# nayuki/DEFLATE-library-Java

Measured on AMD Instinct MI355X. Metric: input MiB/s (compress+decompress), higher is better.
Workload: dtype u8

## Files before the change

deflate-library-java_amd/csrc/capi/ndfl_capi.cpp:

```cpp
#include "../../../include/ndfl.h"
#include "../hip/deflate_kernels.hip"
#include "../hip/deflate_split.hip"
#include "../hip/lz77_kernels.hip"
#include "../hip/strategy_kernels.hip"
#include "../hip/inflate_kernels.hip"

#include <hip/hip_runtime.h>
#include <string.h>
#include <stdio.h>
#include <algorithm>
#include <stdlib.h>
#include <vector>
#include <functional>
#include <map>

namespace {

struct DevBuf {
    void* p = nullptr;
    size_t cap = 0;
    hipError_t ensure(size_t n) {
        if (n <= cap) return hipSuccess;
        if (p) { hipFree(p); p = nullptr; cap = 0; }
        size_t want = n < 4096 ? 4096 : n;
// ... 229 lines not shown
    HIPCHK(c->d_status.ensure(nch * sizeof(uint64_t)));
    HIPCHK(c->d_ticket.ensure(64));
    HIPCHK(c->d_edge_w.ensure(2ull * nch * sizeof(uint64_t)));
    HIPCHK(c->d_edge_v.ensure(2ull * nch * sizeof(uint32_t)));
    if (crc_inout) { HIPCHK(c->d_crc.ensure(nch * sizeof(uint32_t))); HIPCHK(c->d_crc1.ensure(64)); }
    HIPCHK(hipMemsetAsync(c->d_status.p, 0, nch * sizeof(uint64_t), s));
    HIPCHK(hipMemsetAsync(c->d_ticket.p, 0, 64, s));

    Args a;
    a.in = d_data; a.n = len; a.chunk_len = chunk_len; a.nchunks = nch;
    a.prev_byte = prev_byte; a.hist_enabled = hist_limit > 0; a.final_last = final_flag ? 1 : 0;
    a.rle = rle; a.dynamic = dyn; a.base_bit = start_bitpos;
    a.parent_len = c->parent_len ? c->parent_len : chunk_len;
    a.out = d_out; a.status = c->d_status.as<uint64_t>(); a.ticket = c->d_ticket.as<uint32_t>();
    a.edge_w = c->d_edge_w.as<uint64_t>(); a.edge_v = c->d_edge_v.as<uint32_t>();
    a.chunk_bits = c->cb_out;
    a.crc_raw = crc_inout ? c->d_crc.as<uint32_t>() : nullptr;
    a.crc_tab = c->d_tabs.as<uint32_t>();
    a.crc_x = c->d_tabs.as<uint32_t>() + 1024;
    a.prof = nullptr;
    const bool prof = c->knobs.deflate_profile;
    if (prof) { HIPCHK(hipMalloc(&a.prof, (size_t)nch * 128)); HIPCHK(hipMemsetAsync(a.prof, 0, (size_t)nch * 128, s)); }
    a.hist_out = nullptr; a.codes = nullptr; a.chunk_off = nullptr;
    {
        static int ncu = 0;
        if (!ncu && hipDeviceGetAttribute(&ncu, hipDeviceAttributeMultiprocessorCount, c->device) != hipSuccess) ncu = 0;
        a.pf_dist = c->knobs.deflate_pf ? 2u * (uint32_t)ncu : 0u;
    }
    const bool split = !c->knobs.deflate_fused && !prof;
    uint64_t* d_total = nullptr;
    if (split) {
        HIPCHK(c->d_hist.ensure((size_t)nch * HREC * 4));
        HIPCHK(c->d_codes.ensure((size_t)nch * CREC * 4));
        HIPCHK(c->d_off.ensure((size_t)nch * 8 + 64 + (size_t)((nch + SCAN_TILE - 1) / SCAN_TILE) * 8));
        a.hist_out = c->d_hist.as<uint32_t>();
        a.codes = c->d_codes.as<uint32_t>();
        a.chunk_off = c->d_off.as<uint64_t>();
        d_total = c->d_off.as<uint64_t>() + nch;
    }
    a.c0 = 0;
    HIPCHK(hipEventRecord(c->ev0, s));
    if (split) {
        hipLaunchKernelGGL(ndfl_deflate_hist_kernel, dim3(nch), dim3(1024), 0, s, a);
        HIPCHK(hipGetLastError());
        hipLaunchKernelGGL(ndfl_deflate_codes_kernel, dim3(nch), dim3(64), 0, s, a);
        HIPCHK(hipGetLastError());
        const uint32_t ntile = (nch + SCAN_TILE - 1) / SCAN_TILE;
        uint64_t* d_part = c->d_off.as<uint64_t>() + nch + 8;
        hipLaunchKernelGGL(ndfl_deflate_offsets_sum_kernel, dim3(ntile), dim3(SCAN_T), 0, s, (const uint64_t*)a.status,
                           nch, d_part);
        HIPCHK(hipGetLastError());
        hipLaunchKernelGGL(ndfl_deflate_offsets_kernel, dim3(ntile), dim3(SCAN_T), 0, s, (const uint64_t*)a.status, nch,
                           (uint64_t)start_bitpos, c->d_off.as<uint64_t>(), d_total, (const uint64_t*)d_part);
        HIPCHK(hipGetLastError());
        hipLaunchKernelGGL(ndfl_deflate_emit_kernel, dim3(nch), dim3(1024), 0, s, a);
    } else {
        hipLaunchKernelGGL(ndfl_deflate_chunks_kernel, dim3(nch), dim3(1024), 0, s, a);
    }
    HIPCHK(hipGetLastError());
    HIPCHK(hipEventRecord(c->ev1, s));
    const uint32_t ne = 2 * nch;
    hipLaunchKernelGGL(ndfl_edge_fixup_kernel, dim3((ne + 255) / 256), dim3(256), 0, s,
                       (const uint64_t*)a.edge_w, (const uint32_t*)a.edge_v, ne, d_out);
    HIPCHK(hipGetLastError());
    if (crc_inout) {
        HIPCHK(launch_crc_combine(c, s, (const uint32_t*)a.crc_raw, nch, chunk_len, len, c->d_crc1.as<uint32_t>()));
        HIPCHK(hipMemcpyAsync(c->h_pinned + 4, c->d_crc1.p, 4, hipMemcpyDeviceToHost, s));
    }
    if (split) HIPCHK(hipMemcpyAsync(c->h_pinned, d_total, 8, hipMemcpyDeviceToHost, s));
    else HIPCHK(hipMemcpyAsync(c->h_pinned, a.status + (nch - 1), 8, hipMemcpyDeviceToHost, s));
    HIPCHK(hipStreamSynchronize(s));
    float ms = 0;
    hipEventElapsedTime(&ms, c->ev0, c->ev1);
    c->last_ms = ms;
    c->deflate_ms = ms;
    if (prof) {
        std::vector<uint64_t> h((size_t)nch * 16);
        HIPCHK(hipMemcpy(h.data(), a.prof, (size_t)nch * 128, hipMemcpyDeviceToHost));
        hipFree(a.prof);
        double sum[7] = {0}, tmin = 1e300, tmax = 0, sub[6] = {0};
        uint64_t nsub = 0;
        for (uint32_t k = 0; k < nch; k++) {
            const uint64_t* q = &h[k * 16];
            for (int p = 0; p < 7; p++) sum[p] += (double)(q[p + 1] - q[p]);
            tmin = std::min(tmin, (double)q[0]); tmax = std::max(tmax, (double)q[7]);
            if (q[8]) {
                const uint64_t t[7] = {q[2], q[8], q[9], q[10], q[11], q[12], q[13]};
                for (int p = 0; p < 6; p++) sub[p] += (double)(t[p + 1] - t[p]);
                nsub++;
            }
        }
        if (nsub)
            fprintf(stderr, "[ndfl] deflate codes sub-phases (us/chunk): trim %.2f pm(lit,dist) %.2f canon %.2f cl-rle %.2f "
                    "pm(cl) %.2f canon(cl) %.2f\n", sub[0] / nsub / 100, sub[1] / nsub / 100, sub[2] / nsub / 100,
                    sub[3] / nsub / 100, sub[4] / nsub / 100, sub[5] / nsub / 100);
        fprintf(stderr, "[ndfl] deflate phases (us/chunk): load+crc %.2f hist %.2f codes %.2f bits+scan %.2f emit %.2f "
                "lookback %.2f store %.2f; span %.2f ms\n", sum[0] / nch / 100, sum[1] / nch / 100, sum[2] / nch / 100,
                sum[3] / nch / 100, sum[4] / nch / 100, sum[5] / nch / 100, sum[6] / nch / 100, (tmax - tmin) / 1e5);
    }
    uint64_t st;
    memcpy(&st, c->h_pinned, 8);
    const uint64_t end_bits = st & ST_VAL;
    *out_end_bits = end_bits;
    const uint64_t nbytes = (end_bits + 7) / 8;
    if (crc_inout) {
        uint32_t raw = c->h_pinned[4];
        uint32_t dc = ~(crc_multmodp(crc_x8n(len), 0xFFFFFFFFu) ^ raw);
        *crc_inout = ndfl_crc32_combine(*crc_inout, dc, len);
    }
// ... 673 lines not shown
```

deflate-library-java_amd/csrc/hip/deflate_kernels.hip:

```cpp
#include "ndfl_common.hpp"

namespace {

constexpr int DT = 1024;
constexpr int NW = DT / 64;
constexpr int MAX_CHUNK = 65536;
constexpr int OUTW = 18600;

constexpr uint64_t ST_AGG = 1ull << 62;
constexpr uint64_t ST_PRE = 2ull << 62;
constexpr uint64_t ST_VAL = (1ull << 62) - 1;

constexpr int SCR_HLIT = 0;
constexpr int SCR_HDIST = SCR_HLIT + 288 * 4;
constexpr int SCR_LAST = SCR_HDIST + 32 * 4;
constexpr int SCR_KEY = SCR_LAST + 1024;
constexpr int SCR_LF = SCR_KEY + 288 * 4;
constexpr int SCR_LS = SCR_LF + 288 * 4;
constexpr int SCR_PFA = SCR_LS + 288 * 4;
constexpr int SCR_PFB = SCR_PFA + 304 * 4;
constexpr int SCR_MF = SCR_PFB + 304 * 4;
constexpr int SCR_MPK = SCR_MF + 608 * 4;
constexpr int SCR_LVL = SCR_MPK + 15 * 20 * 4;
constexpr int SCR_LEN = SCR_LVL + 16 * 4;
// ... 415 lines not shown

__device__ __forceinline__ void block_store(const uint32_t* obuf, uint64_t P, uint64_t S, uint32_t c, uint32_t* out,
                                            uint64_t* edge_w, uint32_t* edge_v) {
    const int tid = threadIdx.x;
    const uint32_t sh = (uint32_t)(P & 31);
    const uint32_t nw = (uint32_t)((sh + S + 31) >> 5);
    const uint64_t W0 = P >> 5;
    auto outw = [&](uint32_t k) -> uint32_t {
        const uint32_t cur = obuf[k];
        const uint32_t prv = k ? obuf[k - 1] : 0u;
        return sh ? (cur << sh) | (prv >> (32 - sh)) : cur;
    };
    for (uint32_t k = (uint32_t)tid + 1; k + 1 < nw; k += DT) out[W0 + k] = outw(k);
    if (tid == 0) {
        edge_w[2 * c] = W0;
        edge_v[2 * c] = outw(0);
        edge_w[2 * c + 1] = W0 + nw - 1;
        edge_v[2 * c + 1] = nw > 1 ? outw(nw - 1) : 0u;
    }
}

}

template <int MODE, class PS>
__device__ __forceinline__ void deflate_chunk(const Args& a, uint32_t* obuf, PS& ps, uint32_t* hl4 = nullptr,
                                              uint32_t* ctab = nullptr) {
    char* scr = (char*)obuf;
    uint32_t* hlit = (uint32_t*)(scr + SCR_HLIT);
    uint32_t* hdist = (uint32_t*)(scr + SCR_HDIST);
    uint8_t* lastb = (uint8_t*)(scr + SCR_LAST);
    uint32_t* misc = (uint32_t*)(scr + SCR_MISC);

    const int tid = threadIdx.x;
    const int lane = tid & 63, wid = tid >> 6;

    const uint64_t tp0 = wall_clock64();
    if (MODE == MODE_FUSED) {
        if (tid == 0) ps.chunk = atomicAdd(a.ticket, 1u);
    } else {
        if (tid == 0) ps.chunk = a.c0 + blockIdx.x;
    }
    if (MODE == MODE_FUSED) {
        if (tid < 288) hlit[tid] = 0;
        if (tid < 32) hdist[tid] = 0;
    } else if (MODE == MODE_HIST) {
        for (int k = tid; k < HCOPY * HSTR; k += DT) hl4[k] = 0;
        if (a.crc_raw) ctab[tid] = a.crc_tab[tid];
    }
    __syncthreads();
    const uint32_t c = ps.chunk;
    const uint64_t cs = (uint64_t)c * a.chunk_len;
    const uint32_t len_c = (uint32_t)min((uint64_t)a.chunk_len, a.n - cs);
    const bool is_final = a.final_last && (c + 1 == a.nchunks);
    const uint8_t* src = a.in + cs;

    uint32_t w[16];
    const uint32_t t0 = (uint32_t)tid * 64;
    const int vcnt = (int)min(64u, len_c > t0 ? len_c - t0 : 0u);
    if (vcnt == 64 && (((uintptr_t)(src + t0)) & 15) == 0) {
        const u32x4* p = (const u32x4*)(src + t0);
#pragma unroll
        for (int k = 0; k < 4; k++) {
            u32x4 v = __builtin_nontemporal_load(p + k);
            w[4 * k] = v.x; w[4 * k + 1] = v.y; w[4 * k + 2] = v.z; w[4 * k + 3] = v.w;
        }
    } else {
#pragma unroll
        for (int k = 0; k < 16; k++) {
            uint32_t x = 0;
#pragma unroll
            for (int b = 0; b < 4; b++) {
                int i = 4 * k + b;
                if (i < vcnt) x |= (uint32_t)src[t0 + i] << (8 * b);
            }
            w[k] = x;
        }
    }
    if (vcnt > 0) {
        uint32_t lv = w[15] >> 24;
        if (vcnt < 64) {
#pragma unroll
            for (int i = 0; i < 64; i++) if (i == vcnt - 1) lv = (w[i >> 2] >> (8 * (i & 3))) & 0xFFu;
// ... 20 lines not shown
#pragma unroll
            for (int i = 0; i < 64; i++)
                if (i >= nfull * 4 && i < vcnt) cr = T0[(cr ^ (w[i >> 2] >> (8 * (i & 3)))) & 0xFF] ^ (cr >> 8);
        }
        uint32_t contrib = 0;
        if (vcnt > 0) {
            const uint32_t after = len_c - (t0 + (uint32_t)vcnt);
            const uint32_t q = after & 63, k64 = after >> 6;
            uint32_t sh = a.crc_x[64 + k64];
            if (q) sh = crc_multmodp(a.crc_x[q], sh);
            contrib = crc_multmodp(sh, cr);
        }
        contrib = wave_xor(contrib);
        if (lane == 0) ps.crcAcc[wid] = contrib;
    }
    __syncthreads();
    if (MODE != MODE_EMIT && a.crc_raw && tid == 0) {
        uint32_t x = 0;
        for (int k = 0; k < NW; k++) x ^= ps.crcAcc[k];
        a.crc_raw[c] = x;
    }

    const uint64_t tp1 = wall_clock64();
    uint32_t pfv = 0;
    auto prefetch_next = [&]() {
        const uint64_t cn = (uint64_t)c + a.pf_dist;
        if (a.pf_dist && cn < a.nchunks && tid < 512) {
            const uint64_t off = cn * a.chunk_len + (uint64_t)tid * 128;
            if (off < a.n) pfv = a.in[off];
        }
    };
    const bool has_prev0 = (cs % a.parent_len != 0) ? true : (c > 0) ? (a.hist_enabled != 0) : (a.prev_byte >= 0);
    const uint32_t prev0 = (c > 0) ? (uint32_t)src[-1] : (uint32_t)(a.prev_byte & 0xFF);
    uint64_t F = 0;
    if (vcnt > 0) {
        uint32_t prev = tid > 0 ? (uint32_t)lastb[tid - 1] : 0u;
        if (!a.rle) {
            F = vcnt == 64 ? ~0ull : ((1ull << vcnt) - 1);
        } else {
#pragma unroll
            for (int k = 0; k < 16; k++) {
                const uint32_t x = w[k] ^ ((w[k] << 8) | (k ? (w[k - 1] >> 24) : prev));
                const uint32_t hb = ((((x & 0x7F7F7F7Fu) + 0x7F7F7F7Fu) | x) & 0x80808080u) >> 7;
                F |= (uint64_t)(((hb * 0x00204081u) >> 21) & 0xFu) << (4 * k);
            }
            if (tid == 0) F |= 1ull;
            if (vcnt < 64) F &= (1ull << vcnt) - 1;
        }
    }
    const uint32_t firstStart = F ? t0 + (uint32_t)__builtin_ctzll(F) : 0xFFFFFFFFu;
    const uint32_t nextStart = min(block_excl_suffix_min<NW>(firstStart, 0xFFFFFFFFu, ps.scan32), len_c);

    auto lead_of = [&](uint32_t gpos, uint32_t v) -> uint32_t {
        if (!a.rle) return 1u;
        if (gpos == 0) return (has_prev0 && prev0 == v) ? 0u : 1u;
        return 1u;
    };
    uint32_t mpx = 0xFFFFu;
    if (vcnt > 0) {
        mpx = nextStart - t0;
        if (a.rle && tid == 0 && (F & 1) && lead_of(0, w[0] & 0xFFu) == 0) mpx |= 1u << 31;
    }
    uint64_t LM = 0, LG = 0;
    uint32_t ce = 0;
    if (vcnt > 0) {
        const uint32_t mq = mpx & 0xFFFFu;
        const uint64_t wl = F | (mq < 64 ? 1ull << mq : 0ull);
        const uint64_t wh = (mq >= 64 && mq < 67) ? 1ull << (mq - 64) : 0ull;
        const uint64_t e1 = (wl >> 1) | (wh << 63), e2 = (wl >> 2) | (wh << 62), e3 = (wl >> 3) | (wh << 61);
        uint64_t r3 = F & ~e1 & ~e2 & e3;
        LG = F & ~(e1 | e2 | e3);
        if ((mpx >> 31) && (r3 & 1ull)) { r3 &= ~1ull; LG |= 1ull; }
        const uint64_t r2 = (F & ~e1 & e2) | r3;
        const uint64_t r1 = (F & e1) | r2;
        LM = r1 | (r2 << 1) | (r3 << 2);
        ce = (uint32_t)(r2 >> 63) + (uint32_t)((r3 >> 62) & 1ull) + (uint32_t)(r3 >> 63);
    }
#define NDFL_FOR_GROUPS_L(...)                                                                         \
    _Pragma("unroll 1") for (int o_ = 0; o_ < 8; o_++) {                                               \
        const uint32_t lm_ = (uint32_t)(LM >> (8 * o_)) & 0xFFu;                                      \
        const uint32_t lg_ = (uint32_t)(LG >> (8 * o_)) & 0xFFu;                                      \
        if (!__any((lm_ | lg_) != 0)) continue;                                                        \
        const bool o1_ = o_ & 1, o2_ = o_ & 2, o4_ = o_ & 4;                                           \
        const uint32_t a0_ = o1_ ? w[2] : w[0], a1_ = o1_ ? w[6] : w[4];                               \
        const uint32_t a2_ = o1_ ? w[10] : w[8], a3_ = o1_ ? w[14] : w[12];                            \
        const uint32_t b0_ = o1_ ? w[3] : w[1], b1_ = o1_ ? w[7] : w[5];                               \
        const uint32_t b2_ = o1_ ? w[11] : w[9], b3_ = o1_ ? w[15] : w[13];                            \
        const uint32_t gw0_ = o4_ ? (o2_ ? a3_ : a2_) : (o2_ ? a1_ : a0_);                             \
        const uint32_t gw1_ = o4_ ? (o2_ ? b3_ : b2_) : (o2_ ? b1_ : b0_);                             \
        const bool anyL_ = __any(lg_ != 0);                                                            \
        __VA_ARGS__                                                                                    \
    }
#define NDFL_BYTE(j) ((((j) < 4 ? gw0_ : gw1_) >> (8 * ((j) & 3))) & 0xFFu)
#define NDFL_LMASK(j) ((uint32_t)((int32_t)(lm_ << (31 - (j))) >> 31))
#define NDFL_RUN_L(j, ...)                                                                             \
    if ((lg_ >> (j)) & 1) {                                                                            \
        const int i_ = 8 * o_ + (j);                                                                   \
        const uint32_t v = NDFL_BYTE(j);                                                               \
        const uint32_t gpos = t0 + (uint32_t)i_;                                                       \
        const uint64_t rest_ = i_ < 63 ? (F >> (i_ + 1)) : 0ull;                                       \
        const uint32_t pend = rest_ ? gpos + 1 + (uint32_t)__builtin_ctzll(rest_) : nextStart;         \
        __VA_ARGS__                                                                                    \
    }

    uint32_t* hl = hlit;
    uint32_t* hd = hdist;
    if (MODE == MODE_HIST) { hl = hl4 + (tid & (HCOPY - 1)) * HSTR; hd = hl + 288; }
    if (MODE == MODE_HIST) {
        asm volatile("" :: "v"(prev0));
        prefetch_next();
    }
    if (MODE != MODE_EMIT) {
    NDFL_FOR_GROUPS_L({
_Pragma("unroll")
        for (int j = 0; j < 8; j++)
            if ((lm_ >> j) & 1) atomicAdd(&hl[NDFL_BYTE(j)], 1u);
        if (!anyL_) continue;
_Pragma("unroll")
        for (int j = 0; j < 8; j++) {
            NDFL_RUN_L(j, {
                const uint32_t lead = lead_of(gpos, v);
                const uint32_t R = pend - gpos - lead;
                const uint32_t n258 = R / 258, m = R % 258;
                const uint32_t nlit = lead + (m < 3 ? m : 0);
                if (nlit) atomicAdd(&hl[v], nlit);
                if (n258) atomicAdd(&hl[285], n258);
                uint32_t nd = n258;
                if (m >= 3) {
                    uint32_t sym, ne, ex; run_sym(m, sym, ne, ex);
                    atomicAdd(&hl[sym], 1u);
                    nd++;
                }
                if (nd) atomicAdd(&hd[0], nd);
            })
        }
    })
    if (ce) atomicAdd(&hl[w[15] >> 24], ce);
    if (tid == 0) {
        atomicAdd(&hl[256], 1u);
        if (a.dynamic && len_c == 0) atomicAdd(&hl[0], 1u);
    }
    __syncthreads();
    }
    if (MODE == MODE_HIST) {
        uint32_t* h = a.hist_out + (uint64_t)c * HREC;
        if (tid < HREC) {
            uint32_t v = 0;
_Pragma("unroll")
            for (int k = 0; k < HCOPY; k++) v += hl4[k * HSTR + tid];
            h[tid] = v;
        }
        asm volatile("" :: "v"(pfv));
        return;
    }

    const uint64_t tp2 = wall_clock64();
    uint32_t packedLo = 0, packedHi = 0;
    if constexpr (MODE == MODE_FUSED) {
        build_block_codes(a.dynamic != 0, scr, ps, a.prof ? a.prof + (uint64_t)c * 16 + 8 : nullptr);
        packedLo = misc[4]; packedHi = misc[5];
    } else {
        const uint32_t* rec = a.codes + (uint64_t)c * CREC;
        if (tid < 288) ps.litCode[tid] = rec[CREC_LIT + tid];
        else if (tid < 320) ps.distCode[tid - 288] = rec[CREC_DIST + tid - 288];
        if (tid == 0) ps.hdrBits = rec[CREC_META];
    }
    __syncthreads();

    const uint64_t tp3 = wall_clock64();
    if (MODE == MODE_EMIT) prefetch_next();
    const uint32_t d0 = __builtin_amdgcn_readfirstlane(ps.distCode[0]);
    const uint32_t c285 = __builtin_amdgcn_readfirstlane(ps.litCode[285]);
    uint32_t mybits = 0;
    NDFL_FOR_GROUPS_L({
// ... 110 lines not shown
    __syncthreads();

    const uint64_t tp5e = wall_clock64();
    if constexpr (MODE == MODE_FUSED) block_lookback(c, a.base_bit, S, a.status, ps);
    const uint64_t tp5 = wall_clock64();
    const uint64_t P = MODE == MODE_FUSED ? ps.P : a.chunk_off[c];
    block_store(obuf, P, S, c, a.out, a.edge_w, a.edge_v);
    if (tid == 0) {
        if (a.prof) {
            uint64_t* q = a.prof + (uint64_t)c * 16;
            q[0] = tp0; q[1] = tp1; q[2] = tp2; q[3] = tp3; q[4] = tp4; q[5] = tp5e; q[6] = tp5;
            q[7] = wall_clock64();
            (void)tp3a; (void)tp3b;
        }
    }
    (void)is_final; (void)packedLo; (void)packedHi;
    asm volatile("" :: "v"(pfv));
}

extern "C" __global__ void __launch_bounds__(DT, 8)
ndfl_deflate_chunks_kernel(Args a) {
    __shared__ __attribute__((aligned(16))) uint32_t obuf[OUTW];
    __shared__ Persist ps;
    deflate_chunk<MODE_FUSED>(a, obuf, ps);
}

extern "C" __global__ void __launch_bounds__(DT, 8)
ndfl_deflate_hist_kernel(Args a) {
    __shared__ __attribute__((aligned(16))) uint32_t obuf[(SCR_LAST + 1024) / 4];
    __shared__ __attribute__((aligned(16))) uint32_t hl4[HCOPY * HSTR];
    __shared__ uint32_t ctab[1024];
    __shared__ PersistS ps;
    deflate_chunk<MODE_HIST>(a, obuf, ps, hl4, ctab);
}

extern "C" __global__ void __launch_bounds__(DT, 8)
ndfl_deflate_emit_kernel(Args a) {
    __shared__ __attribute__((aligned(16))) uint32_t obuf[OUTW];
    __shared__ PersistS ps;
    deflate_chunk<MODE_EMIT>(a, obuf, ps);
}

extern "C" __global__ void ndfl_edge_fixup_kernel(const uint64_t* edge_w, const uint32_t* edge_v, uint32_t n_edges,
                                                  uint32_t* out) {
    uint32_t e = blockIdx.x * blockDim.x + threadIdx.x;
    if (e >= n_edges) return;
    uint64_t wv = edge_w[e];
    if (e > 0 && edge_w[e - 1] == wv) return;
    uint32_t v = 0;
    for (uint32_t k = e; k < n_edges && edge_w[k] == wv; k++) v |= edge_v[k];
    out[wv] = v;
}

extern "C" __global__ void __launch_bounds__(256)
ndfl_crc_combine_kernel(const uint32_t* crc_raw, uint32_t nchunks, uint32_t chunk_len, uint64_t n,
                        const uint32_t* x8p2, uint32_t* out_raw) {
    uint32_t acc = 0;
    for (uint32_t c = blockIdx.x * blockDim.x + threadIdx.x; c < nchunks; c += gridDim.x * blockDim.x) {
        const uint64_t end = min((uint64_t)(c + 1) * chunk_len, n);
        uint64_t after = n - end;
        uint32_t p = 1u << 31;
        for (int k = 0; after; k++, after >>= 1)
            if (after & 1) p = crc_multmodp(x8p2[k], p);
// ... 83 lines not shown
```

deflate-library-java_amd/csrc/hip/inflate_kernels.hip:

```cpp
#pragma once
#include "ndfl_common.hpp"
#include "../../../include/ndfl.h"
#include <vector>
#include <algorithm>
#include <unordered_map>
#include <chrono>
#include <string.h>
#include <stdio.h>
#include <stdlib.h>

namespace inf {

constexpr uint32_t SEG_BYTES = 65536;
constexpr uint32_t SEG_CAP = 256;
constexpr uint64_t NONE = ~0ull;

enum : uint32_t { ST_BOUNDARY = 0, ST_FINAL = 1, ST_ERROR = 2 };
constexpr int NEED_INPUT = 64;
enum : int { R_UEOS = 1, R_RESERVED_BLOCK_TYPE, R_LEN_MISMATCH, R_UNDER_FULL, R_OVER_FULL, R_NO_PREV,
             R_CL_OVER_FULL, R_EOB_ZERO, R_RESERVED_LEN, R_RESERVED_DIST, R_EMPTY_DIST, R_COPY_BEFORE,
             R_RESERVED_LEN_HI = 20, R_RESERVED_DIST_HI = 21,
             R_INTERNAL = 100 };

constexpr int CLO[19] = {16, 17, 18, 0, 8, 7, 9, 6, 10, 5, 11, 4, 12, 3, 13, 2, 14, 1, 15};
// ... 365 lines not shown
            const uint64_t p = (tw0 + lw) * 32 + o;
            if (ks == 128 && p + 17 + 3 * ncl <= nbits) {
                uint32_t k = atomicAdd(ncand, 1u);
                if (k < FIND_CCAP) cand[k] = (uint32_t)(p - pb) | (1u << 31);
                else find_spill(p | (1ull << 63), qlist, qcount, qcap);
            }
        }
        __builtin_amdgcn_wave_barrier();
    }
}
__device__ __forceinline__ void kr4_fill(uint16_t* kr4) {
    for (uint32_t i = threadIdx.x; i < 4096; i += blockDim.x) {
        uint32_t s = 0;
#pragma unroll
        for (int f = 0; f < 4; f++) { const uint32_t l = (i >> (3 * f)) & 7u; s += l ? 128u >> l : 0u; }
        kr4[i] = (uint16_t)s;
    }
}

}

extern "C" __global__ void __launch_bounds__(256) __attribute__((amdgpu_waves_per_eu(NDFL_FIND_WPE)))
ndfl_inflate_find_compact_kernel(const uint32_t* w, uint64_t nwords, uint64_t nbits, uint64_t* qlist, uint32_t* qcount,
                                 uint32_t qcap, uint64_t w_lo, uint64_t scan_end) {
    using namespace inf;
    __shared__ uint32_t cand[FIND_CCAP];
    __shared__ uint32_t ncand, gbase;
    __shared__ uint16_t kr4[4096];
    __shared__ FindWaveScratch fws[4];
    kr4_fill(kr4);
    if (threadIdx.x == 0) ncand = 0;
    __syncthreads();
    In in{w, nwords, nbits};
    const uint64_t pb = (w_lo + (uint64_t)blockIdx.x * FIND_WPT * 256) * 32;
    for (uint32_t kk = 0; kk < FIND_WPT; kk++) {
        const uint64_t tt = ((uint64_t)blockIdx.x * FIND_WPT + kk) * blockDim.x + threadIdx.x;
        find_word_wave(in, w_lo + tt, scan_end, cand, &ncand, fws[threadIdx.x >> 6], kr4, pb, qlist, qcount, qcap);
    }
    __syncthreads();
    const uint32_t nc = min(ncand, FIND_CCAP);
    if (threadIdx.x == 0) gbase = nc ? atomicAdd(qcount, nc) : 0u;
    __syncthreads();
    for (uint32_t k = threadIdx.x; k < nc; k += blockDim.x) {
        const uint32_t c = cand[k];
        if (gbase + k < qcap) qlist[gbase + k] = (pb + (c & 0x7FFFFFFFu)) | ((uint64_t)(c >> 31) << 63);
    }
}

namespace inf {
struct SRd {
    uint64_t bb, pos, qw;
    uint32_t bn, fi;
    u32x4 cur, nxt;
    __device__ __forceinline__ static uint32_t pick(const u32x4& v, uint32_t i) {
        uint32_t a = (i & 1) ? v.y : v.x, b = (i & 1) ? v.w : v.z;
        return (i & 2) ? b : a;
    }
    __device__ __forceinline__ uint32_t pick8(uint32_t i) const {
        const uint32_t a = pick(cur, i), b = pick(nxt, i);
        return (i & 4) ? b : a;
    }
    __device__ __forceinline__ void load(const In& in, uint64_t g) {
        qw = g;
        cur = in.ld4(g);
        nxt = in.ld4(g + 1);
    }
    __device__ __forceinline__ uint64_t bits64(uint32_t o) const {
        const uint32_t i = o >> 5, sh = o & 31;
// ... 1071 lines not shown
    const uint64_t qtop = std::min<uint64_t>(0x7FFFFFFFull, std::max(qbase, Q_BUDGET));
    uint32_t qcap = (uint32_t)std::max(qbase, std::min<uint64_t>(S.q_min, qtop));
    S.q_full = qcap >= qtop;
    if (inf_ensure(&S.d_q, &S.d_q_cap, (uint64_t)qcap * 8 + 64) != hipSuccess) {
        (void)hipGetLastError();
        qcap = (uint32_t)qbase;
        S.q_full = true;
        S.q_min = 0;
        INF_CHK(inf_ensure(&S.d_q, &S.d_q_cap, (uint64_t)qcap * 8 + 64));
    }
    S.q_cap = qcap;
    uint32_t* d_qcount = (uint32_t*)S.d_stats + SW_QCOUNT;
    uint64_t* d_qlist = (uint64_t*)((char*)S.d_q + 64);
    static const uint32_t strict_grid = [] {
        int dev = 0, ncu = 0, per = 0;
        if (hipGetDevice(&dev) != hipSuccess ||
            hipDeviceGetAttribute(&ncu, hipDeviceAttributeMultiprocessorCount, dev) != hipSuccess ||
            hipOccupancyMaxActiveBlocksPerMultiprocessor(&per, ndfl_inflate_strict_kernel, 256, 0) != hipSuccess ||
            ncu <= 0 || per <= 0)
            return 1280u;
        return (uint32_t)(ncu * per);
    }();
    unsigned long long* sst = S.knobs.stats ? (unsigned long long*)((uint32_t*)S.d_stats + SW_STRICT64) : nullptr;
    if (nw32) {
        const uint32_t fgrid = (uint32_t)((nw32 + 256 * FIND_WPT - 1) / (256 * FIND_WPT));
        hipLaunchKernelGGL(ndfl_inflate_find_compact_kernel, dim3(fgrid), dim3(256), 0, s, d_w, nwords, nbits, d_qlist,
                           d_qcount, qcap, w_lo, scan_end);
        INF_CHK(hipGetLastError());
        hipLaunchKernelGGL(ndfl_inflate_strict_kernel, dim3(strict_grid), dim3(256), 0, s, d_w, nwords, nbits,
                           (const uint64_t*)d_qlist, (const uint32_t*)d_qcount, qcap, d_cnt, d_list,
                           (uint32_t*)S.d_stats + SW_STRICT_TICKET, sst);
        INF_CHK(hipGetLastError());
    }
    return 0;
}

static int inflate_headers(InflateScratch& S, hipStream_t s, const uint8_t* in, uint64_t in_len, uint32_t flags,
                           uint64_t* out, uint64_t cap, uint64_t* n_out, uint64_t* surv, uint64_t surv_cap,
                           uint64_t* stats) {
    using namespace inf;
    const uint64_t nbits = in_len * 8, nwords = (in_len + 3) / 4;
    const uint32_t* d_w = nullptr;
    INF_RC(stage_input(S, s, in, in_len, flags, &d_w));
    if (!S.d_stats) INF_CHK(hipMalloc(&S.d_stats, 512));
    const uint32_t nseg = (uint32_t)std::max<uint64_t>(1, (in_len + SEG_BYTES - 1) / SEG_BYTES);
    INF_CHK(inf_ensure(&S.d_cand, &S.d_cand_cap, (uint64_t)nseg * SEG_CAP * 8ull + (uint64_t)nseg * 4 + 64));
    uint64_t* d_list = (uint64_t*)S.d_cand;
    uint32_t* d_cnt = (uint32_t*)((char*)S.d_cand + (uint64_t)nseg * SEG_CAP * 8ull);
    std::vector<uint32_t> cnt(nseg);
    std::vector<uint64_t> lists((uint64_t)nseg * SEG_CAP);
// ... 446 lines not shown
```

deflate-library-java_amd/csrc/hip/inflate_records.hpp:

```cpp
#pragma once

enum : uint32_t {
    SW_NSLOW = 0, SW_NFIX = 1, SW_NROUND = 2,
    SW_QCOUNT = 8,
    SW_STRICT_TICKET = 10,
    SW_REC_CTR = 12, SW_TREC_CTR = 13,
    SW_TAIL_FAIL = 14,
    SW_STRICT64 = 16,
    SW_CLOCK64 = 32,
};
enum : uint32_t {
    CT_TICKET = 0,
    CT_NFLAT = 4,
    CT_FLAT_REDO = 5,
    CT_FLAT_TIME64 = 6,
    CT_NORD = 8,
    CT_FLAT_WHY = 10,
    CT_ORDER = 16,
};

namespace wv {

constexpr uint32_t LB = 10;
constexpr uint32_t DB = 8;
constexpr uint32_t LX = 320;
constexpr uint32_t DX = 64;
struct Tabs {
// ... 130 lines not shown
```

deflate-library-java_amd/csrc/hip/ndfl_common.hpp:

```cpp
#pragma once
#include <hip/hip_runtime.h>
#include <stdint.h>
#include <stdio.h>
#include <stdlib.h>
#include <string.h>

struct Knobs {
    bool stats = false;
    bool host_times = false;
    bool host_link = false;
    bool no_hdrrec = false;
    bool emit_fast = true;
    bool no_bt = false;
    bool no_alias = false;
    uint32_t count_w = 0;
    bool deflate_pf = true;
    bool deflate_profile = false;
    bool deflate_fused = false;
    bool lz_stats = false;
    bool lz_chain = false;
    int lz_lead = -1;
    bool flat = true;
    uint32_t flat_min = 49152;
    bool test_segflip = false;
    void read() {
        auto on = [](const char* n) { const char* e = getenv(n); return e && strcmp(e, "0") != 0; };
        auto num = [](const char* n, int dflt) { const char* e = getenv(n); return e ? atoi(e) : dflt; };
        stats = on("NDFL_STATS"); host_times = on("NDFL_HOST_TIMES"); host_link = on("NDFL_HOST_LINK");
        no_hdrrec = on("NDFL_NO_HDRREC");
        emit_fast = num("NDFL_EMIT_FAST", 1) != 0;
        no_bt = on("NDFL_NO_BT"); no_alias = on("NDFL_NO_ALIAS");
        count_w = (uint32_t)num("NDFL_COUNT_W", 0);
        deflate_pf = num("NDFL_DEFLATE_PF", 1) != 0; deflate_profile = on("NDFL_DEFLATE_PROFILE");
        deflate_fused = on("NDFL_DEFLATE_FUSED");
        lz_stats = on("NDFL_LZ_STATS");
        const char* se = getenv("NDFL_LZ_SEARCH");
        lz_chain = se && !strcmp(se, "chain");
        lz_lead = num("NDFL_LZ_LEAD", -1);
        test_segflip = on("NDFL_TEST_SEGFLIP");
        flat = num("NDFL_FLAT", 1) != 0;
        flat_min = (uint32_t)num("NDFL_FLAT_MIN", 49152);
    }
    void print(FILE* f) const {
        fprintf(f, "[ndfl] context knobs: stats=%d host_times=%d host_link=%d no_hdrrec=%d emit_fast=%d no_bt=%d "
                   "no_alias=%d count_w=%u deflate_pf=%d deflate_profile=%d deflate_fused=%d lz_stats=%d "
                   "lz_search=%s lz_lead=%d test_segflip=%d flat=%d flat_min=%u\n",
                (int)stats, (int)host_times, (int)host_link, (int)no_hdrrec, (int)emit_fast, (int)no_bt,
                (int)no_alias, count_w, (int)deflate_pf, (int)deflate_profile, (int)deflate_fused, (int)lz_stats,
                lz_chain ? "chain" : "parse", lz_lead, (int)test_segflip, (int)flat, flat_min);
    }
};

#define NDFL_WAVE 64

typedef uint32_t u32x4 __attribute__((ext_vector_type(4)));

#define NDFL_CRC_POLY 0xEDB88320u

__host__ __device__ inline uint32_t crc_multmodp(uint32_t a, uint32_t b) {
    uint32_t m = 1u << 31, p = 0;
    for (;;) {
        if (a & m) {
            p ^= b;
            if ((a & (m - 1)) == 0) break;
        }
        m >>= 1;
        b = (b & 1) ? (b >> 1) ^ NDFL_CRC_POLY : b >> 1;
    }
    return p;
}

__host__ __device__ inline uint32_t crc_x8n(uint64_t n) {
// ... 67 lines not shown
template <class Ld, class St>
__device__ __forceinline__ void scan_tile_apply(Ld ld, St st, uint32_t n, const uint64_t* part, uint64_t init,
                                                uint64_t* grand) {
    __shared__ uint64_t sh[SCAN_T / 64], sp[SCAN_T / 64];
    uint64_t p = 0;
    for (uint32_t t = threadIdx.x; t < blockIdx.x; t += SCAN_T) p += part[t];
    uint64_t before;
    block_excl_scan<uint64_t, SCAN_T / 64>(p, sp, before);
    const uint32_t i0 = blockIdx.x * SCAN_TILE + threadIdx.x * SCAN_PER;
    uint64_t x[SCAN_PER], v = 0;
#pragma unroll
    for (uint32_t k = 0; k < SCAN_PER; k++) x[k] = ld(min(i0 + k, n - 1));
#pragma unroll
    for (uint32_t k = 0; k < SCAN_PER; k++) { if (i0 + k >= n) x[k] = 0; v += x[k]; }
    uint64_t tot;
    uint64_t run = init + before + block_excl_scan<uint64_t, SCAN_T / 64>(v, sh, tot);
#pragma unroll
    for (uint32_t k = 0; k < SCAN_PER; k++)
        if (i0 + k < n) { st(i0 + k, run); run += x[k]; }
    if (grand && blockIdx.x + 1 == gridDim.x && threadIdx.x == 0) *grand = init + before + tot;
}

template <int NWAVES>
__device__ inline uint32_t block_excl_suffix_min(uint32_t v, uint32_t ident, uint32_t* sh) {
    const int lane = threadIdx.x & 63, wid = threadIdx.x >> 6;
    uint32_t x = v;
#pragma unroll
    for (int o = 1; o < 64; o <<= 1) {
        uint32_t y = __shfl_down(x, o, 64);
        if (lane + o < 64) x = min(x, y);
    }
    if (lane == 0) sh[wid] = x;
    __syncthreads();
    uint32_t after = ident;
    for (int w = wid + 1; w < NWAVES; w++) after = min(after, sh[w]);
    uint32_t nxt = __shfl_down(x, 1, 64);
    uint32_t r = (lane == 63) ? after : min(nxt, after);
    __syncthreads();
    return r;
}

__device__ inline uint64_t ld_agent(const uint64_t* p) {
    return __hip_atomic_load(p, __ATOMIC_RELAXED, __HIP_MEMORY_SCOPE_AGENT);
}
__device__ inline void st_agent(uint64_t* p, uint64_t v) {
    __hip_atomic_store(p, v, __ATOMIC_RELAXED, __HIP_MEMORY_SCOPE_AGENT);
}
```

Baseline: 212,900.

## Make deflate hist and inflate find kernels persistent with ticket-based work stealing

The deflate histogram kernel now launches only as many workgroups as are resident (twice the CU count) and loops over chunks taken from an atomic ticket. It zeroes its shared tables once per workgroup and loads the next chunk's input words into registers while the current histogram runs. The inflate find/compact kernel likewise becomes persistent, grabbing tiles through a ticket counter and flushing candidates once per tile. This removes per-workgroup launch and setup overhead and overlaps loads with compute, at the cost of extra register pressure and a dependence on the ticket counters being zeroed; profiling mode no longer forces the fused path.

New measurement: 211,800. Within noise of the previous version (-0.6%).

```diff
diff --git a/deflate-library-java_amd/csrc/capi/ndfl_capi.cpp b/deflate-library-java_amd/csrc/capi/ndfl_capi.cpp
--- a/deflate-library-java_amd/csrc/capi/ndfl_capi.cpp
+++ b/deflate-library-java_amd/csrc/capi/ndfl_capi.cpp
@@ -275,12 +275,13 @@
     const bool prof = c->knobs.deflate_profile;
     if (prof) { HIPCHK(hipMalloc(&a.prof, (size_t)nch * 128)); HIPCHK(hipMemsetAsync(a.prof, 0, (size_t)nch * 128, s)); }
     a.hist_out = nullptr; a.codes = nullptr; a.chunk_off = nullptr;
-    {
-        static int ncu = 0;
-        if (!ncu && hipDeviceGetAttribute(&ncu, hipDeviceAttributeMultiprocessorCount, c->device) != hipSuccess) ncu = 0;
-        a.pf_dist = c->knobs.deflate_pf ? 2u * (uint32_t)ncu : 0u;
-    }
-    const bool split = !c->knobs.deflate_fused && !prof;
+    static int ncu = 0;
+    if (!ncu && hipDeviceGetAttribute(&ncu, hipDeviceAttributeMultiprocessorCount, c->device) != hipSuccess) ncu = 0;
+    const uint32_t resident = ncu > 0 ? 2u * (uint32_t)ncu : 512u;
+    a.pf_dist = c->knobs.deflate_pf && ncu > 0 ? resident : 0u;
+    uint32_t hist_grid = std::min(nch, resident);
+    if (c->knobs.deflate_wgs) hist_grid = std::min(hist_grid, c->knobs.deflate_wgs);
+    const bool split = !c->knobs.deflate_fused;
     uint64_t* d_total = nullptr;
     if (split) {
         HIPCHK(c->d_hist.ensure((size_t)nch * HREC * 4));
@@ -294,7 +295,7 @@
     a.c0 = 0;
     HIPCHK(hipEventRecord(c->ev0, s));
     if (split) {
-        hipLaunchKernelGGL(ndfl_deflate_hist_kernel, dim3(nch), dim3(1024), 0, s, a);
+        hipLaunchKernelGGL(ndfl_deflate_hist_kernel, dim3(hist_grid), dim3(1024), 0, s, a);
         HIPCHK(hipGetLastError());
         hipLaunchKernelGGL(ndfl_deflate_codes_kernel, dim3(nch), dim3(64), 0, s, a);
         HIPCHK(hipGetLastError());
@@ -331,13 +332,28 @@
         std::vector<uint64_t> h((size_t)nch * 16);
         HIPCHK(hipMemcpy(h.data(), a.prof, (size_t)nch * 128, hipMemcpyDeviceToHost));
         hipFree(a.prof);
+        if (split) {
+            auto pass = [&](const char* name, int i0, int i1, int i2, uint32_t wgs) {
+                double res = 0, ld = 0, t0 = 1e300, t1 = 0;
+                for (uint32_t k = 0; k < nch; k++) {
+                    const uint64_t* q = &h[k * 16];
+                    res += (double)(q[i2] - q[i0]); ld += (double)(q[i1] - q[i0]);
+                    t0 = std::min(t0, (double)q[i0]); t1 = std::max(t1, (double)q[i2]);
+                }
+                fprintf(stderr, "[ndfl] deflate %s pass: residency %.2f us/chunk, start to data %.2f us, span %.3f ms, "
+                        "%u workgroup slots, idle share %.3f\n", name, res / nch / 100, ld / nch / 100, (t1 - t0) / 1e5,
+                        wgs, 1.0 - res / ((t1 - t0) * wgs));
+            };
+            pass("hist", 8, 9, 10, hist_grid);
+            pass("emit", 0, 1, 7, std::min(nch, resident));
+        }
         double sum[7] = {0}, tmin = 1e300, tmax = 0, sub[6] = {0};
         uint64_t nsub = 0;
         for (uint32_t k = 0; k < nch; k++) {
             const uint64_t* q = &h[k * 16];
             for (int p = 0; p < 7; p++) sum[p] += (double)(q[p + 1] - q[p]);
             tmin = std::min(tmin, (double)q[0]); tmax = std::max(tmax, (double)q[7]);
-            if (q[8]) {
+            if (!split && q[8]) {
                 const uint64_t t[7] = {q[2], q[8], q[9], q[10], q[11], q[12], q[13]};
                 for (int p = 0; p < 6; p++) sub[p] += (double)(t[p + 1] - t[p]);
                 nsub++;
diff --git a/deflate-library-java_amd/csrc/hip/deflate_kernels.hip b/deflate-library-java_amd/csrc/hip/deflate_kernels.hip
--- a/deflate-library-java_amd/csrc/hip/deflate_kernels.hip
+++ b/deflate-library-java_amd/csrc/hip/deflate_kernels.hip
@@ -461,42 +461,49 @@
 
 }
 
+struct ChunkWords {
+    uint32_t w[16];
+    bool ok;
+    uint32_t next;
+};
+
 template <int MODE, class PS>
-__device__ __forceinline__ void deflate_chunk(const Args& a, uint32_t* obuf, PS& ps, uint32_t* hl4 = nullptr,
-                                              uint32_t* ctab = nullptr) {
+__device__ __forceinline__ void deflate_chunk(const Args& a, uint32_t* obuf, PS& ps, ChunkWords& cw, uint32_t* hl4 = nullptr,
+                                              uint32_t* ctab = nullptr, uint32_t hc = 0, uint32_t hgrid = 0) {
     char* scr = (char*)obuf;
     uint32_t* hlit = (uint32_t*)(scr + SCR_HLIT);
     uint32_t* hdist = (uint32_t*)(scr + SCR_HDIST);
     uint8_t* lastb = (uint8_t*)(scr + SCR_LAST);
     uint32_t* misc = (uint32_t*)(scr + SCR_MISC);
 
-    const int tid = threadIdx.x;
+    int tid = threadIdx.x;
+    if (MODE == MODE_HIST) asm volatile("" : "+v"(tid));
     const int lane = tid & 63, wid = tid >> 6;
 
     const uint64_t tp0 = wall_clock64();
     if (MODE == MODE_FUSED) {
         if (tid == 0) ps.chunk = atomicAdd(a.ticket, 1u);
+    } else if (MODE == MODE_EMIT) {
+        if (tid == 0) ps.chunk = a.c0 + blockIdx.x;
     } else {
-        if (tid == 0) ps.chunk = a.c0 + blockIdx.x;
+        if (tid == 0) ps.chunk = (uint32_t)min((uint64_t)a.c0 + hgrid + atomicAdd(a.ticket, 1u), (uint64_t)0xFFFFFFFFu);
     }
     if (MODE == MODE_FUSED) {
         if (tid < 288) hlit[tid] = 0;
         if (tid < 32) hdist[tid] = 0;
-    } else if (MODE == MODE_HIST) {
-        for (int k = tid; k < HCOPY * HSTR; k += DT) hl4[k] = 0;
-        if (a.crc_raw) ctab[tid] = a.crc_tab[tid];
-    }
-    __syncthreads();
-    const uint32_t c = ps.chunk;
+    }
+    if (MODE != MODE_HIST) __syncthreads();
+    const uint32_t c = MODE == MODE_HIST ? hc : ps.chunk;
     const uint64_t cs = (uint64_t)c * a.chunk_len;
     const uint32_t len_c = (uint32_t)min((uint64_t)a.chunk_len, a.n - cs);
     const bool is_final = a.final_last && (c + 1 == a.nchunks);
     const uint8_t* src = a.in + cs;
 
-    uint32_t w[16];
+    uint32_t (&w)[16] = cw.w;
     const uint32_t t0 = (uint32_t)tid * 64;
     const int vcnt = (int)min(64u, len_c > t0 ? len_c - t0 : 0u);
-    if (vcnt == 64 && (((uintptr_t)(src + t0)) & 15) == 0) {
+    if (MODE == MODE_HIST && cw.ok) {
+    } else if (vcnt == 64 && (((uintptr_t)(src + t0)) & 15) == 0) {
         const u32x4* p = (const u32x4*)(src + t0);
 #pragma unroll
         for (int k = 0; k < 4; k++) {
@@ -563,6 +570,7 @@
     }
 
     const uint64_t tp1 = wall_clock64();
+    if (MODE == MODE_HIST && a.prof && tid == 0) { a.prof[(uint64_t)c * 16 + 8] = tp0; a.prof[(uint64_t)c * 16 + 9] = tp1; }
     uint32_t pfv = 0;
     auto prefetch_next = [&]() {
         const uint64_t cn = (uint64_t)c + a.pf_dist;
@@ -590,7 +598,7 @@
         }
     }
     const uint32_t firstStart = F ? t0 + (uint32_t)__builtin_ctzll(F) : 0xFFFFFFFFu;
-    const uint32_t nextStart = min(block_excl_suffix_min<NW>(firstStart, 0xFFFFFFFFu, ps.scan32), len_c);
+    const uint32_t nextStart = min(block_excl_suffix_min<NW>(firstStart, 0xFFFFFFFFu, ps.scan32, tid), len_c);
 
     auto lead_of = [&](uint32_t gpos, uint32_t v) -> uint32_t {
         if (!a.rle) return 1u;
@@ -632,6 +640,19 @@
         const bool anyL_ = __any(lg_ != 0);                                                            \
         __VA_ARGS__                                                                                    \
     }
+#define NDFL_FOR_GROUPS_HALF(H, ...)                                                                   \
+    _Pragma("unroll 1") for (int o_ = 4 * (H); o_ < 4 * (H) + 4; o_++) {                               \
+        const uint32_t lm_ = (uint32_t)(LM >> (8 * o_)) & 0xFFu;                                      \
+        const uint32_t lg_ = (uint32_t)(LG >> (8 * o_)) & 0xFFu;                                      \
+        if (!__any((lm_ | lg_) != 0)) continue;                                                        \
+        const bool o1_ = o_ & 1, o2_ = o_ & 2;                                                         \
+        const uint32_t a0_ = o1_ ? w[8 * (H) + 2] : w[8 * (H)], a1_ = o1_ ? w[8 * (H) + 6] : w[8 * (H) + 4];       \
+        const uint32_t b0_ = o1_ ? w[8 * (H) + 3] : w[8 * (H) + 1], b1_ = o1_ ? w[8 * (H) + 7] : w[8 * (H) + 5];   \
+        const uint32_t gw0_ = o2_ ? a1_ : a0_;                                                         \
+        const uint32_t gw1_ = o2_ ? b1_ : b0_;                                                         \
+        const bool anyL_ = __any(lg_ != 0);                                                            \
+        __VA_ARGS__                                                                                    \
+    }
 #define NDFL_BYTE(j) ((((j) < 4 ? gw0_ : gw1_) >> (8 * ((j) & 3))) & 0xFFu)
 #define NDFL_LMASK(j) ((uint32_t)((int32_t)(lm_ << (31 - (j))) >> 31))
 #define NDFL_RUN_L(j, ...)                                                                             \
@@ -646,37 +667,64 @@
 
     uint32_t* hl = hlit;
     uint32_t* hd = hdist;
+    const uint32_t wlast = w[15] >> 24;
     if (MODE == MODE_HIST) { hl = hl4 + (tid & (HCOPY - 1)) * HSTR; hd = hl + 288; }
+#define NDFL_HIST_GROUP {                                                                              \
+        _Pragma("unroll")                                                                              \
+        for (int j = 0; j < 8; j++)                                                                    \
+            if ((lm_ >> j) & 1) atomicAdd(&hl[NDFL_BYTE(j)], 1u);                                      \
+        if (!anyL_) continue;                          \
+        _Pragma("unroll")                                                                              \
+        for (int j = 0; j < 8; j++) {                                                                  \
+            NDFL_RUN_L(j, {                                                                            \
+                const uint32_t lead = lead_of(gpos, v);                                                \
+                const uint32_t R = pend - gpos - lead;                                                 \
+                const uint32_t n258 = R / 258, m = R % 258;                                            \
+                const uint32_t nlit = lead + (m < 3 ? m : 0);                                          \
+                if (nlit) atomicAdd(&hl[v], nlit);                                                     \
+                if (n258) atomicAdd(&hl[285], n258);                                                   \
+                uint32_t nd = n258;                                                                    \
+                if (m >= 3) {                                                                          \
+                    uint32_t sym, ne, ex; run_sym(m, sym, ne, ex);                                     \
+                    atomicAdd(&hl[sym], 1u);                                                           \
+                    nd++;                                                                              \
+                }                                                                                      \
+                if (nd) atomicAdd(&hd[0], nd);                                                         \
+            })                                                                                         \
+        }                                                                                              \
+    }
     if (MODE == MODE_HIST) {
         asm volatile("" :: "v"(prev0));
-        prefetch_next();
-    }
+        const uint32_t cn = __builtin_amdgcn_readfirstlane(ps.chunk);
+        cw.next = cn;
+        const uint8_t* sn = a.in;
+        cw.ok = false;
+        if (cn < a.nchunks) {
+            const uint64_t csn = (uint64_t)cn * a.chunk_len;
+            const uint32_t len_n = (uint32_t)min((uint64_t)a.chunk_len, a.n - csn);
+            sn = a.in + csn;
+            cw.ok = len_n >= t0 + 64 && (((uintptr_t)sn) & 15) == 0;
+            if (cw.ok) pfv = *(const uint32_t*)(sn + t0);
+        }
+#define NDFL_NEXT_LOADS(k0)                                                                            \
+        if (cw.ok) {                                                                                  \
+            _Pragma("unroll")                                                                          \
+            for (int k = (k0); k < (k0) + 2; k++) {                                                    \
+                u32x4 v = __builtin_nontemporal_load((const u32x4*)(sn + t0) + k);                     \
+                cw.w[4 * k] = v.x; cw.w[4 * k + 1] = v.y; cw.w[4 * k + 2] = v.z; cw.w[4 * k + 3] = v.w;   \
+            }                                                                                          \
+        }
+        NDFL_FOR_GROUPS_HALF(1, NDFL_HIST_GROUP)
+        NDFL_NEXT_LOADS(2)
+        NDFL_FOR_GROUPS_HALF(0, NDFL_HIST_GROUP)
+        NDFL_NEXT_LOADS(0)
+#undef NDFL_NEXT_LOADS
+    } else if (MODE != MODE_EMIT) {
+        NDFL_FOR_GROUPS_L(NDFL_HIST_GROUP)
+    }
+#undef NDFL_HIST_GROUP
     if (MODE != MODE_EMIT) {
-    NDFL_FOR_GROUPS_L({
-_Pragma("unroll")
-        for (int j = 0; j < 8; j++)
-            if ((lm_ >> j) & 1) atomicAdd(&hl[NDFL_BYTE(j)], 1u);
-        if (!anyL_) continue;
-_Pragma("unroll")
-        for (int j = 0; j < 8; j++) {
-            NDFL_RUN_L(j, {
-                const uint32_t lead = lead_of(gpos, v);
-                const uint32_t R = pend - gpos - lead;
-                const uint32_t n258 = R / 258, m = R % 258;
-                const uint32_t nlit = lead + (m < 3 ? m : 0);
-                if (nlit) atomicAdd(&hl[v], nlit);
-                if (n258) atomicAdd(&hl[285], n258);
-                uint32_t nd = n258;
-                if (m >= 3) {
-                    uint32_t sym, ne, ex; run_sym(m, sym, ne, ex);
-                    atomicAdd(&hl[sym], 1u);
-                    nd++;
-                }
-                if (nd) atomicAdd(&hd[0], nd);
-            })
-        }
-    })
-    if (ce) atomicAdd(&hl[w[15] >> 24], ce);
+    if (ce) atomicAdd(&hl[wlast], ce);
     if (tid == 0) {
         atomicAdd(&hl[256], 1u);
         if (a.dynamic && len_c == 0) atomicAdd(&hl[0], 1u);
@@ -688,9 +736,10 @@
         if (tid < HREC) {
             uint32_t v = 0;
 _Pragma("unroll")
-            for (int k = 0; k < HCOPY; k++) v += hl4[k * HSTR + tid];
+            for (int k = 0; k < HCOPY; k++) { v += hl4[k * HSTR + tid]; hl4[k * HSTR + tid] = 0; }
             h[tid] = v;
         }
+        if (a.prof && tid == 0) a.prof[(uint64_t)c * 16 + 10] = wall_clock64();
         asm volatile("" :: "v"(pfv));
         return;
     }
@@ -847,7 +896,8 @@
 ndfl_deflate_chunks_kernel(Args a) {
     __shared__ __attribute__((aligned(16))) uint32_t obuf[OUTW];
     __shared__ Persist ps;
-    deflate_chunk<MODE_FUSED>(a, obuf, ps);
+    ChunkWords cw;
+    deflate_chunk<MODE_FUSED>(a, obuf, ps, cw);
 }
 
 extern "C" __global__ void __launch_bounds__(DT, 8)
@@ -856,14 +906,22 @@
     __shared__ __attribute__((aligned(16))) uint32_t hl4[HCOPY * HSTR];
     __shared__ uint32_t ctab[1024];
     __shared__ PersistS ps;
-    deflate_chunk<MODE_HIST>(a, obuf, ps, hl4, ctab);
+    for (int k = threadIdx.x; k < HCOPY * HSTR; k += DT) hl4[k] = 0;
+    if (a.crc_raw) ctab[threadIdx.x] = a.crc_tab[threadIdx.x];
+    __syncthreads();
+    ChunkWords cw;
+    cw.ok = false;
+    cw.next = 0;
+    for (uint32_t c = a.c0 + blockIdx.x; c < a.nchunks; c = cw.next)
+        deflate_chunk<MODE_HIST>(a, obuf, ps, cw, hl4, ctab, c, gridDim.x);
 }
 
 extern "C" __global__ void __launch_bounds__(DT, 8)
 ndfl_deflate_emit_kernel(Args a) {
     __shared__ __attribute__((aligned(16))) uint32_t obuf[OUTW];
     __shared__ PersistS ps;
-    deflate_chunk<MODE_EMIT>(a, obuf, ps);
+    ChunkWords cw;
+    deflate_chunk<MODE_EMIT>(a, obuf, ps, cw);
 }
 
 extern "C" __global__ void ndfl_edge_fixup_kernel(const uint64_t* edge_w, const uint32_t* edge_v, uint32_t n_edges,
diff --git a/deflate-library-java_amd/csrc/hip/inflate_kernels.hip b/deflate-library-java_amd/csrc/hip/inflate_kernels.hip
--- a/deflate-library-java_amd/csrc/hip/inflate_kernels.hip
+++ b/deflate-library-java_amd/csrc/hip/inflate_kernels.hip
@@ -411,28 +411,39 @@
 
 extern "C" __global__ void __launch_bounds__(256) __attribute__((amdgpu_waves_per_eu(NDFL_FIND_WPE)))
 ndfl_inflate_find_compact_kernel(const uint32_t* w, uint64_t nwords, uint64_t nbits, uint64_t* qlist, uint32_t* qcount,
-                                 uint32_t qcap, uint64_t w_lo, uint64_t scan_end) {
+                                 uint32_t qcap, uint64_t w_lo, uint64_t scan_end, uint32_t ntiles, uint32_t* ticket) {
     using namespace inf;
     __shared__ uint32_t cand[FIND_CCAP];
-    __shared__ uint32_t ncand, gbase;
+    __shared__ uint32_t ncand, nflush, gbase, next_tile;
     __shared__ uint16_t kr4[4096];
     __shared__ FindWaveScratch fws[4];
     kr4_fill(kr4);
     if (threadIdx.x == 0) ncand = 0;
-    __syncthreads();
     In in{w, nwords, nbits};
-    const uint64_t pb = (w_lo + (uint64_t)blockIdx.x * FIND_WPT * 256) * 32;
-    for (uint32_t kk = 0; kk < FIND_WPT; kk++) {
-        const uint64_t tt = ((uint64_t)blockIdx.x * FIND_WPT + kk) * blockDim.x + threadIdx.x;
-        find_word_wave(in, w_lo + tt, scan_end, cand, &ncand, fws[threadIdx.x >> 6], kr4, pb, qlist, qcount, qcap);
-    }
-    __syncthreads();
-    const uint32_t nc = min(ncand, FIND_CCAP);
-    if (threadIdx.x == 0) gbase = nc ? atomicAdd(qcount, nc) : 0u;
-    __syncthreads();
-    for (uint32_t k = threadIdx.x; k < nc; k += blockDim.x) {
-        const uint32_t c = cand[k];
-        if (gbase + k < qcap) qlist[gbase + k] = (pb + (c & 0x7FFFFFFFu)) | ((uint64_t)(c >> 31) << 63);
+    for (uint32_t tile = blockIdx.x; tile < ntiles;) {
+        __syncthreads();
+        if (threadIdx.x == 0) {
+            const uint64_t nt = (uint64_t)gridDim.x + atomicAdd(ticket, 1u);
+            next_tile = (uint32_t)min(nt, (uint64_t)0xFFFFFFFFu);
+        }
+        const uint64_t pb = (w_lo + (uint64_t)tile * FIND_WPT * 256) * 32;
+        for (uint32_t kk = 0; kk < FIND_WPT; kk++) {
+            const uint64_t tt = ((uint64_t)tile * FIND_WPT + kk) * blockDim.x + threadIdx.x;
+            find_word_wave(in, w_lo + tt, scan_end, cand, &ncand, fws[threadIdx.x >> 6], kr4, pb, qlist, qcount, qcap);
+        }
+        __syncthreads();
+        if (threadIdx.x == 0) {
+            nflush = min(ncand, FIND_CCAP);
+            gbase = nflush ? atomicAdd(qcount, nflush) : 0u;
+            ncand = 0;
+        }
+        __syncthreads();
+        const uint32_t nc = nflush;
+        for (uint32_t k = threadIdx.x; k < nc; k += blockDim.x) {
+            const uint32_t c = cand[k];
+            if (gbase + k < qcap) qlist[gbase + k] = (pb + (c & 0x7FFFFFFFu)) | ((uint64_t)(c >> 31) << 63);
+        }
+        tile = next_tile;
     }
 }
 
@@ -1550,10 +1561,21 @@
         return (uint32_t)(ncu * per);
     }();
     unsigned long long* sst = S.knobs.stats ? (unsigned long long*)((uint32_t*)S.d_stats + SW_STRICT64) : nullptr;
+    static const uint32_t find_grid = [] {
+        int dev = 0, ncu = 0, per = 0;
+        if (hipGetDevice(&dev) != hipSuccess ||
+            hipDeviceGetAttribute(&ncu, hipDeviceAttributeMultiprocessorCount, dev) != hipSuccess ||
+            hipOccupancyMaxActiveBlocksPerMultiprocessor(&per, ndfl_inflate_find_compact_kernel, 256, 0) != hipSuccess ||
+            ncu <= 0 || per <= 0)
+            return 768u;
+        return (uint32_t)(ncu * per);
+    }();
     if (nw32) {
-        const uint32_t fgrid = (uint32_t)((nw32 + 256 * FIND_WPT - 1) / (256 * FIND_WPT));
+        const uint32_t ntiles = (uint32_t)((nw32 + 256 * FIND_WPT - 1) / (256 * FIND_WPT));
+        uint32_t fgrid = std::min(ntiles, find_grid);
+        if (S.knobs.find_wgs) fgrid = std::min(fgrid, S.knobs.find_wgs);
         hipLaunchKernelGGL(ndfl_inflate_find_compact_kernel, dim3(fgrid), dim3(256), 0, s, d_w, nwords, nbits, d_qlist,
-                           d_qcount, qcap, w_lo, scan_end);
+                           d_qcount, qcap, w_lo, scan_end, ntiles, (uint32_t*)S.d_stats + SW_FIND_TICKET);
         INF_CHK(hipGetLastError());
         hipLaunchKernelGGL(ndfl_inflate_strict_kernel, dim3(strict_grid), dim3(256), 0, s, d_w, nwords, nbits,
                            (const uint64_t*)d_qlist, (const uint32_t*)d_qcount, qcap, d_cnt, d_list,
diff --git a/deflate-library-java_amd/csrc/hip/inflate_records.hpp b/deflate-library-java_amd/csrc/hip/inflate_records.hpp
--- a/deflate-library-java_amd/csrc/hip/inflate_records.hpp
+++ b/deflate-library-java_amd/csrc/hip/inflate_records.hpp
@@ -3,6 +3,7 @@
 enum : uint32_t {
     SW_NSLOW = 0, SW_NFIX = 1, SW_NROUND = 2,
     SW_QCOUNT = 8,
+    SW_FIND_TICKET = 9,
     SW_STRICT_TICKET = 10,
     SW_REC_CTR = 12, SW_TREC_CTR = 13,
     SW_TAIL_FAIL = 14,
diff --git a/deflate-library-java_amd/csrc/hip/ndfl_common.hpp b/deflate-library-java_amd/csrc/hip/ndfl_common.hpp
--- a/deflate-library-java_amd/csrc/hip/ndfl_common.hpp
+++ b/deflate-library-java_amd/csrc/hip/ndfl_common.hpp
@@ -4,6 +4,7 @@
 #include <stdio.h>
 #include <stdlib.h>
 #include <string.h>
+#include <algorithm>
 
 struct Knobs {
     bool stats = false;
@@ -14,6 +15,8 @@
     bool no_bt = false;
     bool no_alias = false;
     uint32_t count_w = 0;
+    uint32_t deflate_wgs = 0;
+    uint32_t find_wgs = 0;
     bool deflate_pf = true;
     bool deflate_profile = false;
     bool deflate_fused = false;
@@ -33,6 +36,8 @@
         count_w = (uint32_t)num("NDFL_COUNT_W", 0);
         deflate_pf = num("NDFL_DEFLATE_PF", 1) != 0; deflate_profile = on("NDFL_DEFLATE_PROFILE");
         deflate_fused = on("NDFL_DEFLATE_FUSED");
+        deflate_wgs = (uint32_t)std::max(0, num("NDFL_DEFLATE_WGS", 0));
+        find_wgs = (uint32_t)std::max(0, num("NDFL_FIND_WGS", 0));
         lz_stats = on("NDFL_LZ_STATS");
         const char* se = getenv("NDFL_LZ_SEARCH");
         lz_chain = se && !strcmp(se, "chain");
@@ -44,10 +49,11 @@
     void print(FILE* f) const {
         fprintf(f, "[ndfl] context knobs: stats=%d host_times=%d host_link=%d no_hdrrec=%d emit_fast=%d no_bt=%d "
                    "no_alias=%d count_w=%u deflate_pf=%d deflate_profile=%d deflate_fused=%d lz_stats=%d "
-                   "lz_search=%s lz_lead=%d test_segflip=%d flat=%d flat_min=%u\n",
+                   "lz_search=%s lz_lead=%d test_segflip=%d flat=%d flat_min=%u deflate_wgs=%u find_wgs=%u\n",
                 (int)stats, (int)host_times, (int)host_link, (int)no_hdrrec, (int)emit_fast, (int)no_bt,
                 (int)no_alias, count_w, (int)deflate_pf, (int)deflate_profile, (int)deflate_fused, (int)lz_stats,
-                lz_chain ? "chain" : "parse", lz_lead, (int)test_segflip, (int)flat, flat_min);
+                lz_chain ? "chain" : "parse", lz_lead, (int)test_segflip, (int)flat, flat_min,
+                deflate_wgs, find_wgs);
     }
 };
 
@@ -161,8 +167,8 @@
 }
 
 template <int NWAVES>
-__device__ inline uint32_t block_excl_suffix_min(uint32_t v, uint32_t ident, uint32_t* sh) {
-    const int lane = threadIdx.x & 63, wid = threadIdx.x >> 6;
+__device__ inline uint32_t block_excl_suffix_min(uint32_t v, uint32_t ident, uint32_t* sh, int tid = threadIdx.x) {
+    const int lane = tid & 63, wid = tid >> 6;
     uint32_t x = v;
 #pragma unroll
     for (int o = 1; o < 64; o <<= 1) {
```
